# manycore-research/PlankAssembly

Hardware: AMD Instinct MI355X
Metric: train samples/sec (fwd+bwd+all-reduce+Adam), d_model=512 seq=1024 [value: bf16 MFMA, f32 accumulate / master weights; train.f32 / train.x3: the same step in exact f32 / f32 with bf16x3 products = the parity paths] (higher is better)
Workload: dtype bf16; 1 GPU; train_complete.yaml model d_model=512 H=8 dff=1024 6+6 post-norm layers, dropout 0.2, S=1024 (MAX_INPUT_LENGTH 1025), T=128, batch 16/GPU; global_batch=16, seq_len=1024, parallelism=dp1

## Files before the change

### include/plank_hip.h

```cpp
#ifndef PLANK_HIP_H
#define PLANK_HIP_H
#include <stdint.h>

#ifdef __cplusplus
extern "C" {
#endif

#define PA_F32 0
#define PA_BF16 1

#define PA_EINVAL (-1)
#define PA_EALIGN (-2)
#define PA_ESHAPE (-3)

int pa_version(void);

typedef struct {
    const void* A; const void* B; void* C;
    const float* bias;
    const void* R;
    const void* aux;
    void* ws;
    int32_t M, N, K;
    int32_t lda, ldb, ldc, ldr, ldaux;
// ... 152 lines not shown
                    int32_t dtype, const pa_reduce_desc* rd, int32_t n_rd, void* stream);


typedef struct {
    const void* q; const void* k; const void* v; void* o;
    float* lse;
    const uint8_t* kpm;
    int32_t B, H, Lq, Lk, dh;
    int32_t ldq, ldk, ldv, ldo;
    int32_t causal;
    float scale;
    float drop_p; uint32_t drop_seed;
    int32_t dtype;
    const void* dout; void* dq; void* dk; void* dv; float* delta;
    int32_t lddo, lddq, lddk, lddv;
    const int32_t* cu_q; const int32_t* cu_k;
    const int32_t* order;
    void* ws; int64_t ws_bytes;
} pa_attn_args;
int pa_attn_fwd(const pa_attn_args* a, void* stream);
int pa_attn_bwd(const pa_attn_args* a, void* stream);
int64_t pa_attn_ws_bytes(int32_t rows_total, int32_t B, int32_t H, int32_t L_max);
int64_t pa_attn_ws_ticket_bytes(int64_t ws_bytes);
int pa_attn_split_config(int32_t on);
int64_t pa_attn_split_taken(int32_t reset);

int pa_gelu_fwd(void* out, const void* pre, int64_t rows, int32_t cols, int32_t ld, int32_t dtype, float drop_p, uint32_t drop_seed,
                void* stream);
int pa_gelu_bwd(void* dpre, const void* dh, const void* pre, int64_t rows, int32_t cols, int32_t ld, int32_t dtype, float drop_p,
                uint32_t drop_seed, void* stream);
int pa_switch_fwd(float* s, const void* h, int32_t dtype, const float* w, const float* b, int64_t rows,
                  int32_t d, void* stream);
int pa_switch_bwd(void* dh, int32_t accumulate, float* dw, float* db, const float* ds, const void* h,
                  int32_t dtype, const float* w, float* partial, int64_t rows, int32_t d, void* stream);
int pa_mixture_nll_fwd(float* stats, float* row_lse, const float* vocab, int32_t ldv, const float* ptr,
                       const float* sw, const int64_t* label, int32_t B, int32_t T, int32_t V, int32_t pad,
                       void* stream);
int pa_mixture_nll_bwd(void* dvocab, void* dptr, int32_t out_dtype, float* dsw, const float* stats,
                       const float* row_lse, const float* vocab, int32_t ldv, const float* ptr, const float* sw,
                       const int64_t* label, int32_t B, int32_t T, int32_t V, int32_t pad, float gscale,
                       void* stream);
int pa_mixture_nll_fwd_fin(float* stats8, float* row_lse, const float* vocab, int32_t ldv, const float* ptr,
                           const float* sw, const int64_t* label, int32_t B, int32_t T, int32_t V, int32_t pad,
                           void* stream);
int pa_mixture_nll_bwd_up(void* dvocab, void* dptr, int32_t out_dtype, float* dsw, const float* stats,
                       const float* row_lse, const float* vocab, int32_t ldv, const float* ptr, const float* sw,
// ... 99 lines not shown
```

### plankassembly_amd/_lib.py

```python
from __future__ import annotations

import ctypes as C
import os

import torch

HERE = os.path.dirname(os.path.abspath(__file__))
LIB_PATH = os.environ.get("PLANK_HIP_LIB") or os.path.join(HERE, "libplank_hip.so")

PA_F32, PA_BF16 = 0, 1
_ERR = {-1: "PA_EINVAL (bad argument)", -2: "PA_EALIGN (misaligned pointer / leading dimension)",
        -3: "PA_ESHAPE (unsupported shape)", -4: "PA_ESTATE (bad model/workspace state)"}


class PlankHipError(RuntimeError):
    pass


class GemmArgs(C.Structure):
    _fields_ = [("A", C.c_void_p), ("B", C.c_void_p), ("C", C.c_void_p), ("bias", C.c_void_p),
                ("R", C.c_void_p), ("aux", C.c_void_p), ("ws", C.c_void_p),
                ("M", C.c_int32), ("N", C.c_int32), ("K", C.c_int32),
                ("lda", C.c_int32), ("ldb", C.c_int32), ("ldc", C.c_int32), ("ldr", C.c_int32),
                ("ldaux", C.c_int32),
# ... 104 lines not shown
            "pa_gemm_recorded_kinds": (I, [P, I]),
            "pa_gemm_recorded_groups": (I, [P, I]),
            "pa_splitk_reduce_many": (I, [P, I, P]),
            "pa_colsum_many": (I, [P, I, I, P]),
            "pa_colsum_ws_floats": (I64, [I, I]),
            "pa_colsum": (I, [P, I, I, I, I, P, I, P, P]),
            "pa_embed_input_fwd": (I, [P, I, P, P, P, I, I64, I, P]),
            "pa_embed_input_bwd": (I, [P, I, P, P, P, P, I, I64, I, P]),
            "pa_embed_segment_bwd": (I, [P, I, P, P, P, P, I, I64, I, P]),
            "pa_pack_rows": (I, [P, I, I, P, P, P]),
            "pa_group_rows": (I, [P, I, P]),
            "pa_embed_output_fwd": (I, [P, I, P, P, P, P, I, I, I, I, I, P]),
            "pa_embed_output_bwd": (I, [P, I, P, P, P, P, I, I, I, I, I, P]),
            "pa_layernorm_ws_floats": (I64, [I64, I]),
            "pa_layernorm_fwd": (I, [P, P, P, P, P, P, I64, I, F, I, P]),
            "pa_layernorm_bwd": (I, [P, P, P, P, P, P, P, P, P, P, P, I64, I, I, F, U, P]),
            "pa_layernorm_bwd_partial": (I, [P, P, P, P, P, P, P, I, P, I64, I, I, F, U, P]),
            "pa_layernorm_bwd_nparts": (I, [I64]),
            "pa_layernorm_finish_many": (I, [P, I, I, P]),
            "pa_attn_fwd": (I, [P, P]),
            "pa_attn_bwd": (I, [P, P]),
            "pa_attn_ws_bytes": (I64, [I, I, I, I]),
            "pa_attn_ws_ticket_bytes": (I64, [I64]),
            "pa_attn_split_config": (I, [I]),
            "pa_attn_split_taken": (I64, [I]),
            "pa_gelu_fwd": (I, [P, P, I64, I, I, I, F, C.c_uint32, P]),
            "pa_gelu_bwd": (I, [P, P, P, I64, I, I, I, F, C.c_uint32, P]),
            "pa_switch_fwd": (I, [P, P, I, P, P, I64, I, P]),
            "pa_switch_bwd": (I, [P, I, P, P, P, P, I, P, P, I64, I, P]),
            "pa_mixture_nll_fwd": (I, [P, P, P, I, P, P, P, I, I, I, I, P]),
            "pa_mixture_nll_bwd": (I, [P, P, I, P, P, P, P, I, P, P, P, I, I, I, I, F, P]),
            "pa_mixture_nll_fwd_fin": (I, [P, P, P, I, P, P, P, I, I, I, I, P]),
            "pa_mixture_nll_bwd_up": (I, [P, P, I, P, P, P, P, I, P, P, P, I, I, I, I, F, P, P]),
            "pa_model_set_upstream": (I, [P, P]),
            "pa_adam_step": (I, [P, P, P, P, P, I64, F, F, F, F, I, F, P]),
            "pa_cast": (I, [P, I, P, I, I64, P]),
            "pa_fake_collective": (I, [P, I64, I, I, F, P]),
            "pa_model_create": (I, [P, P]),
            "pa_model_destroy": (None, [P]),
            "pa_model_num_params": (I, [P]),
            "pa_model_bind": (I, [P, P, P, P]),
            "pa_model_bind_transposed": (I, [P, P]),
            "pa_model_bind_cross_kv_t": (I, [P, P]),
            "pa_transpose_many": (I, [P, I, I, I, P]),
            "pa_model_train_ws_bytes": (I64, [P, I, I, I]),
            "pa_model_train_fwd": (I, [P, P, P, I64, U, I, P, P]),
# ... 67 lines not shown
```

### plankassembly_amd/csrc/attention.hip

```cpp
#include <stdio.h>
#include <atomic>
#include <algorithm>
#include "pa_device.h"
#include "../../include/plank_hip.h"

namespace {

constexpr int NTH = 256;
constexpr int BOWN = 128;
constexpr int BSTR = 64;
constexpr float LOG2E = 1.4426950408889634f;
constexpr float LN2 = 0.6931471805599453f;
constexpr float RESCALE_THR = 8.0f;

__device__ __forceinline__ float fast_exp2(float x) { return __builtin_amdgcn_exp2f(x); }

struct AttnP;
struct AttnP {
    const void* q; const void* k; const void* v; void* o; float* lse; const uint8_t* kpm;
    int B, H, Lq, Lk;
    int ldq, ldk, ldv, ldo;
    int causal; float scale;
    uint32_t drop_thr; float drop_scale; uint32_t drop_seed;
    const void* dout; void* dq; void* dk; void* dv; float* delta;
    int lddo, lddq, lddk, lddv;
    const int32_t* cu_q; const int32_t* cu_k;
    const int32_t* order;
    int balanced;
    int ks_min;
    int parts_q, parts_kv;
    int* sp_tick; char* sp_part; int sp_slots, sp_pmax, sp_kmax;
};
constexpr int SP_BYTES = 64 * 1024;

__device__ __forceinline__ AttnP batch_view(const AttnP& pin, int b, int& qoff, int& koff, int off = 0, int len = -1) {
    AttnP p = pin;
    qoff = b * pin.Lq; koff = b * pin.Lk;
    if (len >= 0 && pin.cu_q == pin.cu_k) { qoff = koff = off; p.Lq = p.Lk = len; return p; }
    if (pin.cu_q) { qoff = pin.cu_q[b]; p.Lq = pin.cu_q[b + 1] - qoff; }
    if (pin.cu_k) { koff = pin.cu_k[b]; p.Lk = pin.cu_k[b + 1] - koff; }
    return p;
}

template <typename T, int DH> struct AT {
    static constexpr int EB = ET<T>::EB, KC = ET<T>::KC;
    static constexpr int NS = DH / KC;
    static constexpr int NDT = (DH + 31) / 32;
    static constexpr int NCHR = DH / EB;
    static constexpr int RBN = DH * sizeof(T);
    static constexpr int RBT = BSTR * sizeof(T);
    static constexpr int NCHT = RBT / 16;
    static constexpr int NAT_BYTES = BSTR * RBN;
    static constexpr int TR_BYTES = DH * RBT;
    static constexpr int NSB = 16 * NCHR;
    static constexpr int NITEM = (2 * NSB + NTH - 1) / NTH;
};
// ... 653 lines not shown
    for (int d = 1; d < 64; d <<= 1) { const int v = __shfl_up(sinc, d); if (lane >= d) sinc += v; }
    if (sinc > pin.sp_slots) np = 1;
    const int t = tq * np;
    int inc = t;
#pragma unroll
    for (int d = 1; d < 64; d <<= 1) { const int v = __shfl_up(inc, d); if (lane >= d) inc += v; }
    const int n = __shfl(inc, 63);
    const int row = j >> 5, pos = j & 31, left = n - (row << 5);
    if (left <= 0) return false;
    const int rowlen = left < 32 ? left : 32;
    if (pos >= rowlen) return false;
    const int k = (row << 5) + ((row & 1) ? rowlen - 1 - pos : pos);
    const int rank = __popcll(__ballot(inc <= k));
    const int local = k - (__shfl(inc, rank) - __shfl(t, rank));
    const int npr = __shfl(np, rank);
    u.nparts = __builtin_amdgcn_readfirstlane(npr);
    u.tile = __builtin_amdgcn_readfirstlane(local / npr);
    u.part = __builtin_amdgcn_readfirstlane(local % npr);
    u.b = __builtin_amdgcn_readfirstlane(__shfl(o, rank));
    u.off = __builtin_amdgcn_readfirstlane(__shfl(c0, rank));
    u.len = __builtin_amdgcn_readfirstlane(__shfl(cl, rank));
    u.slot = __builtin_amdgcn_readfirstlane(((__shfl(sinc, rank) - __shfl(spl, rank)) + u.tile) * 8 + x);
    u.h = x;
    return true;
}
#include "split_merge.h"


template <int DH> struct BT {
    static constexpr int RBN = DH * 2;
    static constexpr int NCHR = RBN / 16;
    static constexpr int NAT = BSTR * RBN;
    static constexpr int NCHUNK = BSTR * NCHR;
    static constexpr int NLD = (NCHUNK + NTH - 1) / NTH;
    static constexpr int NS = DH / 16;
    static constexpr int NDT = (DH + 31) / 32;
};

template <int DH>
__device__ __forceinline__ void glds_nat(char* lds, const bf16* base, int ld, int row0, int nrows, int tid, int wave) {
    using B = BT<DH>;
    constexpr int RPB = (B::RBN >= 256) ? 1 : 256 / B::RBN;
#pragma unroll
    for (int i = 0; i < B::NLD; ++i) {
        const int p = tid + i * NTH;
        if (B::NCHUNK % NTH == 0 || p < B::NCHUNK) {
// ... 909 lines not shown
        m_run = m_new;
    }
    const float inv = l_tot > 0.f ? (DROP ? p.drop_scale : 1.0f) / l_tot : 0.f;
    bf16* Op = reinterpret_cast<bf16*>(p.o) + (size_t)qoff * p.ldo + h * DH;
    store_rows4(Op, p.ldo, qrow, p.Lq, oacc, inv, lane);
    if (g == 0 && qrow < p.Lq && p.lse)
        p.lse[((size_t)b * p.H + h) * pin.Lq + qrow] = l_tot > 0.f ? (m_run + log2f(l_tot)) * LN2 : 0.f;
#ifdef PA_ATTN_TRACE
    asm volatile("s_waitcnt vmcnt(0)" ::: "memory");
    PA_TR(4);
    if (tid == 0 && blockIdx.x < 8192) { pa_attn_trace[blockIdx.x * 8 + 5] = nsteps; pa_attn_trace[blockIdx.x * 8 + 6] = __builtin_amdgcn_s_getreg((4 << 0) | (0 << 6) | (31 << 11)); }
#endif
}

template <bool DROP, int KS>
__device__ __forceinline__ void attn4_dq_body(const AttnP& pin, int bid, char* smem) {
    constexpr int DH = 64, NAT = BT<DH>::NAT, BUF = BL<DH>::BUF, AUX = BL<DH>::AUX;
    const int lane = threadIdx.x & 63, g = lane >> 4;
    const int wave_all = __builtin_amdgcn_readfirstlane(threadIdx.x >> 6);
    const int kh = KS == 2 ? (wave_all >> 3) : 0;
    const int wave = wave_all & 7, tid = threadIdx.x & (NT4 - 1);
    int tile_, h, b, off_ = 0, len_ = -1;
    int part = 0, nparts = 1, slot = 0;
    if (KS == 1 && pin.balanced == 2) {
        SplitUnit su;
        if (!decode_unit_split(pin, pin.cu_q, su, bid)) return;
        tile_ = su.tile; h = su.h; b = su.b; off_ = su.off; len_ = su.len; part = su.part; nparts = su.nparts; slot = su.slot;
    }
    else if (pin.balanced) { if (!decode_block_balanced(pin, pin.cu_q, tile_, h, b, off_, len_, bid)) return; }
    else { decode_block((pin.Lq + BOWN - 1) / BOWN, pin.H, pin.B, tile_, h, b, bid); b = dispatch_batch(pin.order, b); }
    int qoff, koff;
    const AttnP p = batch_view(pin, b, qoff, koff, off_, len_);
    const int q0 = tile_ * BOWN;
    if (q0 >= p.Lq) return;
    const bf16* Qp = reinterpret_cast<const bf16*>(p.q) + (size_t)qoff * p.ldq + h * DH;
    const bf16* Kp = reinterpret_cast<const bf16*>(p.k) + (size_t)koff * p.ldk + h * DH;
    const bf16* Vp = reinterpret_cast<const bf16*>(p.v) + (size_t)koff * p.ldv + h * DH;
    const bf16* dOp = reinterpret_cast<const bf16*>(p.dout) + (size_t)qoff * p.lddo + h * DH;
    const uint8_t* mp = p.kpm ? p.kpm + (size_t)b * pin.Lk : nullptr;
    const int qw0 = q0 + wave * 16, qrow = qw0 + (lane & 15);
    const bool wave_on = qw0 < p.Lq;

    u32x4 qreg[2], doreg[2];
    load_row4(qreg, Qp, p.ldq, qrow, p.Lq, lane);
    load_row4(doreg, dOp, p.lddo, qrow, p.Lq, lane);
    scale_row4(qreg, p.scale * LOG2E);
    const size_t srow = ((size_t)b * p.H + h) * pin.Lq + qrow;
    const float lse2 = (qrow < p.Lq) ? p.lse[srow] * LOG2E : INFINITY;
    const float keep_p = DROP ? 1.0f / p.drop_scale : 1.0f;
// ... 94 lines not shown
                if (DROP) dp = drop_keep2(arow, cq[kb & 1][e], p.drop_thr) ? dp : ndlt;
                sacc[kb][e] = pe * dp;
            }
        }
        mma_tr4<buf * BUF>(dqacc, lb, sacc);
        tile_barrier();
    };
    for (int step = 0; step < nsteps; step += 2) {
        body(step, IC<0>{});
        if (step + 1 < nsteps) body(step + 1, IC<1>{});
    }
    if (KS == 2 && split) {
        f32x4* xo = reinterpret_cast<f32x4*>(smem) + wave * 4 * 64;
        if (kh == 1) {
#pragma unroll
            for (int db = 0; db < 4; ++db) xo[db * 64 + lane] = dqacc[db];
        }
        __syncthreads();
        if (kh == 1) return;
#pragma unroll
        for (int db = 0; db < 4; ++db) dqacc[db] += xo[db * 64 + lane];
    }
    if (KS == 1 && nparts > 1) {
        char* const pbase = pin.sp_part + (size_t)slot * pin.sp_pmax * SP_BYTES;
        const SplitOut so(pbase + (size_t)part * SP_BYTES, SP_BYTES);
#pragma unroll
        for (int db = 0; db < 4; ++db) so.put(db, NT4, dqacc[db]);
        if (!split_arrive(pin.sp_tick + slot, nparts, reinterpret_cast<int*>(smem + 2 * BUF))) return;
        for (int pp = 0; pp < nparts; ++pp) {
            if (pp == part) continue;
#pragma unroll
            for (int db = 0; db < 4; ++db) dqacc[db] += split_get(pbase + (size_t)pp * SP_BYTES, db, NT4, SP_BYTES);
        }
    }
    bf16* dQp = reinterpret_cast<bf16*>(p.dq) + (size_t)qoff * p.lddq + h * DH;
    store_rows4(dQp, p.lddq, qrow, p.Lq, dqacc, p.scale * (DROP ? p.drop_scale : 1.0f), lane);
}

template <bool DROP, int KS>
__global__ __launch_bounds__(NT4 * KS, 4) void attn4_bwd_dq_kernel(AttnP pin) {
    extern __shared__ __attribute__((aligned(256))) char smem[];
    attn4_dq_body<DROP, KS>(pin, blockIdx.x, smem);
}

template <bool DROP, bool CAUSAL, bool SELF_DELTA>
__device__ __forceinline__ void attn4_dkv_body(const AttnP& pin, int bid, char* smem) {
    constexpr int DH = 64, NAT = BT<DH>::NAT, BUF = BL<DH>::BUF, AUX = BL<DH>::AUX;
    const int tid = threadIdx.x, lane = tid & 63, g = lane >> 4;
    const int wave = __builtin_amdgcn_readfirstlane(tid >> 6);
    int tile_, h, b, off_ = 0, len_ = -1;
    int part = 0, nparts = 1, slot = 0;
    if (!SELF_DELTA && pin.balanced == 2) {
        SplitUnit su;
        if (!decode_unit_split(pin, pin.cu_k, su, bid)) return;
        tile_ = su.tile; h = su.h; b = su.b; off_ = su.off; len_ = su.len; part = su.part; nparts = su.nparts; slot = su.slot;
// ... 118 lines not shown
                    const bool keep = drop_keep2(aq[e], ckey, p.drop_thr);
                    pd = keep ? pe : 0.f;
                    x = keep ? x : __uint_as_float(nd4[qb][e]);
                }
                sacc[qb][e] = pd;
                dpacc[qb][e] = pe * x;
            }
        }
        mma_tr4<buf * BUF + NAT>(dvacc, lb, sacc);
        mma_tr4<buf * BUF>(dkacc, lb, dpacc);
        if (more) issue_aux(step + 1, buf ^ 1);
        tile_barrier();
    };
    for (int step = step0; step < nsteps; step += 2) {
        body(step, IC<0>{});
        if (step + 1 < nsteps) body(step + 1, IC<1>{});
    }
    if (nparts > 1) {
        char* const pbase = pin.sp_part + (size_t)slot * pin.sp_pmax * SP_BYTES;
        const SplitOut so(pbase + (size_t)part * SP_BYTES, SP_BYTES);
#pragma unroll
        for (int db = 0; db < 4; ++db) { so.put(db, NT4, dkacc[db]); so.put(4 + db, NT4, dvacc[db]); }
        if (!split_arrive(pin.sp_tick + slot, nparts, reinterpret_cast<int*>(smem + 2 * BUF))) return;
        for (int pp = 0; pp < nparts; ++pp) {
            if (pp == part) continue;
#pragma unroll
            for (int db = 0; db < 4; ++db) {
                dkacc[db] += split_get(pbase + (size_t)pp * SP_BYTES, db, NT4, SP_BYTES);
                dvacc[db] += split_get(pbase + (size_t)pp * SP_BYTES, 4 + db, NT4, SP_BYTES);
            }
        }
    }
    bf16* dKp = reinterpret_cast<bf16*>(p.dk) + (size_t)koff * p.lddk + h * DH;
    bf16* dVp = reinterpret_cast<bf16*>(p.dv) + (size_t)koff * p.lddv + h * DH;
    const float ds = DROP ? p.drop_scale : 1.0f;
    store_rows4(dKp, p.lddk, krow, p.Lk, dkacc, kmasked ? 0.f : p.scale * ds, lane, kmasked);
    store_rows4(dVp, p.lddv, krow, p.Lk, dvacc, kmasked ? 0.f : ds, lane, kmasked);
}

template <bool DROP, bool CAUSAL>
__global__ __launch_bounds__(NT4, 4) void attn4_bwd_dkv_kernel(AttnP pin) {
    extern __shared__ __attribute__((aligned(256))) char smem[];
    attn4_dkv_body<DROP, CAUSAL, false>(pin, blockIdx.x, smem);
}
template <bool DROP, bool CAUSAL>
__global__ __launch_bounds__(NT4, 4) void attn4_bwd_merged_kernel(AttnP pin, int gq) {
    extern __shared__ __attribute__((aligned(256))) char smem[];
    if ((int)blockIdx.x < gq) attn4_dq_body<DROP, 1>(pin, blockIdx.x, smem);
    else attn4_dkv_body<DROP, CAUSAL, true>(pin, (int)blockIdx.x - gq, smem);
}

#include "attention5.h"
#include "attention_x3.h"

static int split_kmax() { static const int v = getenv("PA_ATTN_SPLIT_KMAX") ? atoi(getenv("PA_ATTN_SPLIT_KMAX")) : 8; return v < 1 ? 1 : v; }
static int split_pmax() { static const int v = getenv("PA_ATTN_SPLIT_PMAX") ? atoi(getenv("PA_ATTN_SPLIT_PMAX")) : 2; return v < 1 ? 1 : v > 8 ? 8 : v; }
AttnP make_params(const pa_attn_args* a) {
    AttnP p;
    p.q = a->q; p.k = a->k; p.v = a->v; p.o = a->o; p.lse = a->lse; p.kpm = a->kpm;
    p.B = a->B; p.H = a->H; p.Lq = a->Lq; p.Lk = a->Lk;
    p.ldq = a->ldq; p.ldk = a->ldk; p.ldv = a->ldv; p.ldo = a->ldo;
    p.causal = a->causal; p.scale = a->scale;
    p.drop_thr = (uint32_t)((double)a->drop_p * 4294967296.0);
    p.drop_scale = (float)(1.0 / (1.0 - (double)p.drop_thr / 4294967296.0));
    p.drop_seed = a->drop_seed;
    p.dout = a->dout; p.dq = a->dq; p.dk = a->dk; p.dv = a->dv; p.delta = a->delta;
    p.lddo = a->lddo; p.lddq = a->lddq; p.lddk = a->lddk; p.lddv = a->lddv;
    p.cu_q = a->cu_q; p.cu_k = a->cu_k; p.order = a->order;
    static const bool bal_env = !(getenv("PA_ATTN_BALANCED") && atoi(getenv("PA_ATTN_BALANCED")) == 0);
    p.ks_min = 4; p.parts_q = 1; p.parts_kv = 1;
    p.balanced = (bal_env && a->order && a->cu_q && a->cu_k && a->H == 8 && a->B <= 64) ? 1 : 0;
    p.sp_tick = nullptr; p.sp_part = nullptr; p.sp_slots = 0; p.sp_pmax = split_pmax(); p.sp_kmax = split_kmax();
    static const bool sp_env = getenv("PA_ATTN_SPLIT") && atoi(getenv("PA_ATTN_SPLIT")) != 0;
    if (sp_env && p.balanced && a->ws && a->cu_q == a->cu_k && !a->kpm && !a->causal && a->dtype == PA_BF16 && a->dh == 64 &&
        (reinterpret_cast<uintptr_t>(a->ws) & 255) == 0 && p.sp_pmax > 1) {
        const int64_t per = (int64_t)p.sp_pmax * SP_BYTES + 64;
        const int64_t total = a->ws_bytes / per;
        p.sp_slots = (int)(total / 8 < (1 << 20) ? total / 8 : (1 << 20));
        p.sp_tick = static_cast<int*>(a->ws);
        p.sp_part = static_cast<char*>(a->ws) + ((int64_t)p.sp_slots * 8 * 4 + 255) / 256 * 256;
        if ((int64_t)p.sp_slots * 8 * per > a->ws_bytes || p.sp_slots < 1) { p.sp_slots = 0; p.sp_tick = nullptr; }
    }
    return p;
}
static unsigned split_grid(const AttnP& p, int owned_max, int streamed_max) {
    const int ks = (streamed_max + BSTR - 1) / BSTR;
    const int np = ks > p.sp_kmax ? std::min(p.sp_pmax, (ks + p.sp_kmax - 1) / p.sp_kmax) : 1;
    return (unsigned)(8 * p.B * ((owned_max + BOWN - 1) / BOWN) * np);
}

template <typename K> int set_lds(K kern, int bytes) {
    if (bytes > 64 * 1024) {
        hipError_t e = hipFuncSetAttribute(reinterpret_cast<const void*>(kern), hipFuncAttributeMaxDynamicSharedMemorySize, bytes);
        if (e != hipSuccess) return (int)e;
    }
    return 0;
}

static bool use_v4(const AttnP& p, int rows_owned) {
    static const int mode = getenv("PA_ATTN_V4") ? atoi(getenv("PA_ATTN_V4")) : 1;
    if (mode == 0) return false;
    if (mode >= 2) return true;
    const long long waves32 = (long long)p.B * p.H * ((rows_owned + 31) / 32);
    return p.cu_q != nullptr || p.cu_k != nullptr || waves32 < 4 * 1024;
}
// ... 36 lines not shown
                if (p.drop_thr) PA_LAUNCH((attn4_fwd_kernel<true, 2>), grid, dim3(2 * NT4), shm2, st, p);
                else PA_LAUNCH((attn4_fwd_kernel<false, 2>), grid, dim3(2 * NT4), shm2, st, p);
                return 0;
            }
            if (p.drop_thr) PA_LAUNCH((attn4_fwd_kernel<true, 1>), grid, dim3(NT4), shm, st, p);
            else PA_LAUNCH((attn4_fwd_kernel<false, 1>), grid, dim3(NT4), shm, st, p);
            return 0;
        }
    }
    if (p.drop_thr) PA_LAUNCH((attn_fwd_bf16_kernel<DH, true>), grid, dim3(NTH), shm, st, p);
    else PA_LAUNCH((attn_fwd_bf16_kernel<DH, false>), grid, dim3(NTH), shm, st, p);
    return 0;
}
template <int DH> int run_bwd_bf16(AttnP p, hipStream_t st) {
    const int shm = BL<DH>::SHM;
    const dim3 gq0(((p.Lq + BOWN - 1) / BOWN) * p.H * p.B), gk0(((p.Lk + BOWN - 1) / BOWN) * p.H * p.B);
    if constexpr (DH == 64) {
        if (use_v4(p, p.Lq > p.Lk ? p.Lq : p.Lk)) {
            dim3 gq = gq0, gk = gk0;
            static const bool merge_env = !(getenv("PA_ATTN_BWD_MERGE") && atoi(getenv("PA_ATTN_BWD_MERGE")) == 0);
            static const int merge_max = getenv("PA_ATTN_BWD_MERGE_MAX") ? atoi(getenv("PA_ATTN_BWD_MERGE_MAX")) : 128;
            if (merge_env && p.Lq <= merge_max && p.Lq <= 2048 && (gq.x & 7) == 0) {
                const int shm3 = shm + (p.Lq + 15) / 16 * 64 + 64;
                const dim3 gm(gq.x + gk.x);
                if (p.drop_thr) {
                    if (p.causal) PA_LAUNCH((attn4_bwd_merged_kernel<true, true>), gm, dim3(NT4), shm3, st, p, (int)gq.x);
                    else PA_LAUNCH((attn4_bwd_merged_kernel<true, false>), gm, dim3(NT4), shm3, st, p, (int)gq.x);
                } else {
                    if (p.causal) PA_LAUNCH((attn4_bwd_merged_kernel<false, true>), gm, dim3(NT4), shm3, st, p, (int)gq.x);
                    else PA_LAUNCH((attn4_bwd_merged_kernel<false, false>), gm, dim3(NT4), shm3, st, p, (int)gq.x);
                }
                return 0;
            }
            bool ks = use_ksplit(p, gq.x);
            constexpr int shm2 = 4 * BL<DH>::BUF + 64;
            if (p.balanced && p.sp_tick && !ks) { p.balanced = 2; gq = dim3(split_grid(p, p.Lq, p.Lk)); gk = dim3(split_grid(p, p.Lk, p.Lq)); }
            if (ks) {
                static const int rc_d = set_lds(attn4_bwd_dq_kernel<true, 2>, shm2), rc_n = set_lds(attn4_bwd_dq_kernel<false, 2>, shm2);
                if (rc_d || rc_n) return rc_d ? rc_d : rc_n;
            }
            if (p.drop_thr) {
                if (ks) PA_LAUNCH((attn4_bwd_dq_kernel<true, 2>), gq, dim3(2 * NT4), shm2, st, p);
                else PA_LAUNCH((attn4_bwd_dq_kernel<true, 1>), gq, dim3(NT4), shm, st, p);
                if (p.causal) PA_LAUNCH((attn4_bwd_dkv_kernel<true, true>), gk, dim3(NT4), shm, st, p);
                else PA_LAUNCH((attn4_bwd_dkv_kernel<true, false>), gk, dim3(NT4), shm, st, p);
            } else {
                if (ks) PA_LAUNCH((attn4_bwd_dq_kernel<false, 2>), gq, dim3(2 * NT4), shm2, st, p);
                else PA_LAUNCH((attn4_bwd_dq_kernel<false, 1>), gq, dim3(NT4), shm, st, p);
                if (p.causal) PA_LAUNCH((attn4_bwd_dkv_kernel<false, true>), gk, dim3(NT4), shm, st, p);
                else PA_LAUNCH((attn4_bwd_dkv_kernel<false, false>), gk, dim3(NT4), shm, st, p);
            }
            return 0;
        }
    }
    const dim3 gq = gq0, gk = gk0;
    static const int occ_env = getenv("PA_ATTN_OCC") ? atoi(getenv("PA_ATTN_OCC")) : 0;
// ... 108 lines not shown
    if (bwd) {
        if (!a->dout || !a->dq || !a->dk || !a->dv || !a->delta) return PA_EINVAL;
        if (!al(a->dout, a->lddo) || !al(a->dq, a->lddq) || !al(a->dk, a->lddk) || !al(a->dv, a->lddv)) return PA_EALIGN;
    }
    return 0;
}

}

extern "C" int pa_attn_split_config(int32_t on) { return pa_split_attn_set(on); }
extern "C" int64_t pa_attn_split_taken(int32_t reset) {
    const long long v = g_attn_x3_taken.load();
    if (reset) g_attn_x3_taken.store(0);
    return v;
}

extern "C" int64_t pa_attn_ws_bytes(int32_t rows_total, int32_t B, int32_t H, int32_t L_max) {
    static const bool sp_env = getenv("PA_ATTN_SPLIT") && atoi(getenv("PA_ATTN_SPLIT")) != 0;
    if (!sp_env || split_pmax() < 2 || H != 8 || rows_total <= 0 || B <= 0 || B > 64) return 0;
    if ((L_max + BSTR - 1) / BSTR <= split_kmax()) return 0;
    const int64_t slots = (int64_t)(rows_total / BOWN + B);
    return slots * 8 * ((int64_t)split_pmax() * SP_BYTES + 64) + 256;
}
extern "C" int64_t pa_attn_ws_ticket_bytes(int64_t ws_bytes) {
    const int64_t per = (int64_t)split_pmax() * SP_BYTES + 64;
    return (ws_bytes / per / 8 * 8 * 4 + 255) / 256 * 256;
}

extern "C" int pa_attn_fwd(const pa_attn_args* a, void* stream) {
    int rc = check_args(a, false);
    if (rc) return rc;
    hipStream_t st = reinterpret_cast<hipStream_t>(stream);
    return a->dtype == PA_BF16 ? dispatch<bf16>(a, false, st) : dispatch<float>(a, false, st);
}

extern "C" int pa_attn_bwd(const pa_attn_args* a, void* stream) {
    int rc = check_args(a, true);
    if (rc) return rc;
    hipStream_t st = reinterpret_cast<hipStream_t>(stream);
    return a->dtype == PA_BF16 ? dispatch<bf16>(a, true, st) : dispatch<float>(a, true, st);
}

#ifdef PA_ATTN_TRACE
extern "C" int pa_attn_trace_read(unsigned long long* out, int32_t n) {
    return (int)hipMemcpyFromSymbol(out, HIP_SYMBOL(pa_attn_trace), sizeof(unsigned long long) * (size_t)n);
}
// ... 2 lines not shown
```

### plankassembly_amd/csrc/model.h

```cpp
#pragma once
#include <hip/hip_runtime.h>
#include <stdint.h>
#include <vector>
#include "../../include/plank_hip.h"

struct Arena {
    char* base; size_t off;
    void* take(size_t bytes) {
        size_t o = (off + 255) & ~(size_t)255;
        off = o + bytes;
        return base ? base + o : nullptr;
    }
};

static inline uint32_t site_seed(uint32_t base, uint32_t site) {
    uint32_t x = base + 0x9e3779b9u * (site + 1);
    x ^= x >> 16; x *= 0x7feb352du; x ^= x >> 15; x *= 0x846ca68bu; x ^= x >> 16;
    return x;
}

enum { P_IN_VALUE = 0, P_IN_POS, P_IN_COORD, P_IN_VIEW, P_IN_TYPE, P_Q_COORD, P_Q_POS, P_FIXED_HEAD };
enum { E_IN_W = 0, E_IN_B, E_OUT_W, E_OUT_B, E_L1_W, E_L1_B, E_L2_W, E_L2_B, E_N1_W, E_N1_B, E_N2_W, E_N2_B, E_COUNT };
enum { D_SA_IN_W = 0, D_SA_IN_B, D_SA_OUT_W, D_SA_OUT_B, D_CA_IN_W, D_CA_IN_B, D_CA_OUT_W, D_CA_OUT_B,
       D_L1_W, D_L1_B, D_L2_W, D_L2_B, D_N1_W, D_N1_B, D_N2_W, D_N2_B, D_N3_W, D_N3_B, D_COUNT };
// ... 6 lines not shown
    void *qkv, *o_sa, *z1, *y1, *q_ca, *kv_ca, *o_ca, *z2, *y2, *hff, *z3;
    int ld_kv = 0;
    float *lse_sa, *lse_ca, *m1, *r1, *m2, *r2, *m3, *r3;
};

struct DecodeLayout;
struct pa_model {
    pa_model_cfg cfg;
    int n_params;
    std::vector<void*> pf, pl, gr;
    std::vector<void*> plT;
    bool bound = false;
    bool have_fwd = false;
    pa_batch batch;
    int B = 0, S = 0, T = 0;
    int NE = 0;
    uint32_t seed = 0; float p_drop = 0.f;
    size_t esz = 4;
    std::vector<void*> X, Y;
    std::vector<EncAct> ea; std::vector<DecAct> da;
    void *memory = nullptr, *hid = nullptr; float *mem_m = nullptr, *mem_r = nullptr, *hid_m = nullptr, *hid_r = nullptr;
    float *vlog = nullptr, *plog = nullptr, *sw = nullptr, *row_lse = nullptr; void* pfeat = nullptr; int ldv = 0;
    float* stats = nullptr;
    void* attn_ws = nullptr; int64_t attn_ws_bytes = 0; void* attn_ws_zeroed = nullptr; int64_t attn_ws_zeroed_bytes = 0;
    const float* upstream = nullptr;
    void *gA, *gB, *gC, *gD, *gE, *gF, *gQ3, *gKV, *dmem, *dvlog, *dplog; float *dsw, *delta, *partial, *splitws;
    void* gPre = nullptr;
    size_t splitws_floats = 0;
    void* gBs[3] = {nullptr, nullptr, nullptr}; void* gCs[3] = {nullptr, nullptr, nullptr};
    float* lnp[3] = {nullptr, nullptr, nullptr}; pa_ln_finish_desc lnq[PA_MAX_LN_FINISH]; int nlnq = 0;
    pa_gemm_args dwq[PA_MAX_GROUP]; int ndwq = 0;
    pa_colsum_desc cs[PA_MAX_COLSUM]; int ncs = 0; bool defer_ok = false;
    pa_reduce_desc defer[PA_MAX_REDUCE]; int ndefer = 0; size_t slab_used = 0;
    bool dmem_written = false;
    void* kv_all = nullptr;
    void* gKV_all = nullptr; const void* kvT_all = nullptr;
    struct SegSet { void* gBs[3]; void* gCs[3]; void *gE, *gF, *gQ3, *gKV; float* lnp[3]; float* splitws; };
    SegSet seg_set[2];
    void select_set(int par) {
        const SegSet& s = seg_set[par];
        for (int i = 0; i < 3; ++i) { gBs[i] = s.gBs[i]; gCs[i] = s.gCs[i]; lnp[i] = s.lnp[i]; }
        gE = s.gE; gF = s.gF; gQ3 = s.gQ3; gKV = s.gKV; splitws = s.splitws;
    }
    bool side_on = false;
    void* side = nullptr;
    void* ev_ready[2] = {nullptr, nullptr};
    void* ev_done[2] = {nullptr, nullptr};
// ... 12 lines not shown
```

### plankassembly_amd/csrc/runtime.hip

```cpp
#include <stdlib.h>
#include <hip/hip_runtime.h>
#include <math.h>
#include <new>
#include <string.h>
#include <vector>
#include "../../include/plank_hip.h"

#include "model.h"

namespace {

#define RC(x) do { int rc_ = (x); if (rc_) return rc_; } while (0)

struct Ctx {
    pa_model* m; void* st;
    int dt() const { return m->cfg.dtype; }
    bool gelu() const { return m->cfg.activation == 2; }
    int ffn1(const void* A, const void* W, const float* bias, void* hidden, int rows, float drop_p, uint32_t seed) const {
        const int d = m->cfg.d_model, ff = m->cfg.d_ff;
        if (!gelu()) return linear(A, d, W, bias, hidden, ff, rows, ff, d, 1, drop_p, seed);
        RC(linear(A, d, W, bias, hidden, ff, rows, ff, d, 0));
        return pa_gelu_fwd(hidden, hidden, rows, ff, ff, dt(), drop_p, seed, st);
    }

// ... 102 lines not shown
            void* const out = ddrop ? ddrop : dz;
            const bool al = ((reinterpret_cast<uintptr_t>(dz) | reinterpret_cast<uintptr_t>(dy) | reinterpret_cast<uintptr_t>(z) |
                              reinterpret_cast<uintptr_t>(ddrop) | reinterpret_cast<uintptr_t>(g) | reinterpret_cast<uintptr_t>(part)) & 15) == 0;
            void* img = (al && pa_layernorm_bwd_can_img(m->cfg.d_model, dt())) ?
                        pa_gemm_split_reserve(out, (int32_t)rows, m->cfg.d_model, m->cfg.d_model, &pat) : nullptr;
            RC(pa_layernorm_bwd_partial_img(dz, ddrop, dy, z, g, mean, rstd, dzsum ? 1 : 0, part, rows, m->cfg.d_model, dt(), drop_p, seed,
                                            img, pat, st));
            pa_ln_finish_desc& fd = m->lnq[m->nlnq++];
            fd.partial = part; fd.nparts = pa_layernorm_bwd_nparts(rows); fd.pad_ = 0; fd.dgamma = dg; fd.dbeta = db; fd.dzsum = dzsum;
            return 0;
        }
        return pa_layernorm_bwd(dz, ddrop, dy, z, g, mean, rstd, dg, db, dzsum, m->partial, rows, m->cfg.d_model, dt(),
                                drop_p, seed, st);
    }
    int attn(bool bwd, const void* q, int ldq, const void* k, const void* v, int ldkv, void* o, float* lse,
             const uint8_t* kpm, int Lq, int Lk, int causal, float drop_p, uint32_t seed,
             const void* dout = nullptr, void* dq = nullptr, int lddq = 0, void* dk = nullptr, void* dv = nullptr,
             int lddkv = 0, const int32_t* cu_q = nullptr, const int32_t* cu_k = nullptr) const {
        pa_attn_args a; memset(&a, 0, sizeof(a));
        a.cu_q = cu_q; a.cu_k = cu_k;
        static const bool use_order = !(getenv("PA_ATTN_ORDER") && atoi(getenv("PA_ATTN_ORDER")) == 0);
        if (use_order && cu_k && cu_k == m->batch.cu_in) a.order = cu_k + m->B + 1;
        if (cu_q && cu_q == cu_k) { a.ws = m->attn_ws; a.ws_bytes = m->attn_ws_bytes; }
        const int d = m->cfg.d_model, H = m->cfg.n_head;
        a.q = q; a.k = k; a.v = v; a.o = o; a.lse = lse; a.kpm = kpm;
        a.B = m->B; a.H = H; a.Lq = Lq; a.Lk = Lk; a.dh = d / H;
        a.ldq = ldq; a.ldk = ldkv; a.ldv = ldkv; a.ldo = d;
        a.causal = causal; a.scale = 1.0f / sqrtf((float)(d / H));
        a.drop_p = drop_p; a.drop_seed = seed; a.dtype = dt();
        if (!bwd) return pa_attn_fwd(&a, st);
        a.dout = dout; a.dq = dq; a.dk = dk; a.dv = dv; a.delta = m->delta;
        a.lddo = d; a.lddq = lddq; a.lddk = lddkv; a.lddv = lddkv;
        return pa_attn_bwd(&a, st);
    }
};

}
size_t pa_train_layout(pa_model* m, char* base, int B, int S, int T) {
    const pa_model_cfg& c = m->cfg;
    const size_t e = c.dtype == PA_BF16 ? 2 : 4;
    const size_t d = c.d_model, ff = c.d_ff, H = c.n_head;
    const size_t BS = (size_t)B * S, BT = (size_t)B * T, R = BS > BT ? BS : BT;
    Arena a{base, 0};
    m->esz = e;
    {
        const int64_t n = c.dtype == PA_BF16 ? pa_attn_ws_bytes(B * S, B, (int32_t)H, S) : 0;
        m->attn_ws = n > 0 ? a.take((size_t)n) : nullptr;
        m->attn_ws_bytes = n > 0 ? n : 0;
    }
    m->X.resize(c.n_enc + 1); m->Y.resize(c.n_dec + 1); m->ea.resize(c.n_enc); m->da.resize(c.n_dec);
    for (int i = 0; i <= c.n_enc; ++i) m->X[i] = a.take(BS * d * e);
    for (int i = 0; i < c.n_enc; ++i) {
        EncAct& t = m->ea[i];
        t.qkv = a.take(BS * 3 * d * e); t.o = a.take(BS * d * e); t.z1 = a.take(BS * d * e); t.y1 = a.take(BS * d * e);
        t.hff = a.take(BS * ff * e); t.z2 = a.take(BS * d * e);
        t.lse = (float*)a.take((size_t)B * H * S * 4);
        t.m1 = (float*)a.take(BS * 4); t.r1 = (float*)a.take(BS * 4); t.m2 = (float*)a.take(BS * 4); t.r2 = (float*)a.take(BS * 4);
    }
    m->memory = a.take(BS * d * e); m->mem_m = (float*)a.take(BS * 4); m->mem_r = (float*)a.take(BS * 4);
    for (int i = 0; i <= c.n_dec; ++i) m->Y[i] = a.take(BT * d * e);
    for (int i = 0; i < c.n_dec; ++i) {
        DecAct& t = m->da[i];
        t.qkv = a.take(BT * 3 * d * e); t.o_sa = a.take(BT * d * e); t.z1 = a.take(BT * d * e); t.y1 = a.take(BT * d * e);
        t.q_ca = a.take(BT * d * e); t.kv_ca = nullptr; t.o_ca = a.take(BT * d * e);
        t.z2 = a.take(BT * d * e); t.y2 = a.take(BT * d * e); t.hff = a.take(BT * ff * e); t.z3 = a.take(BT * d * e);
        t.lse_sa = (float*)a.take((size_t)B * H * T * 4); t.lse_ca = (float*)a.take((size_t)B * H * T * 4);
        t.m1 = (float*)a.take(BT * 4); t.r1 = (float*)a.take(BT * 4); t.m2 = (float*)a.take(BT * 4);
        t.r2 = (float*)a.take(BT * 4); t.m3 = (float*)a.take(BT * 4); t.r3 = (float*)a.take(BT * 4);
// ... 503 lines not shown

extern "C" int64_t pa_model_train_ws_bytes(pa_model* m, int32_t B, int32_t S, int32_t T) {
    if (!m || B <= 0 || S <= 0 || T <= 0) return PA_EINVAL;
    return (int64_t)pa_train_layout(m, nullptr, B, S, T) + 256;
}

extern "C" int pa_model_train_fwd(pa_model* m, const pa_batch* batch, void* ws, int64_t ws_bytes, uint32_t seed,
                                  int32_t training, float* stats, void* stream) {
    if (!m || !m->bound || !batch || !ws || !stats) return PA_EINVAL;
    if (batch->B <= 0 || batch->S <= 0 || batch->T <= 0 || !batch->input_idx[0] || !batch->input_mask) return PA_EINVAL;
    if (batch->output_value && (!batch->output_label || !batch->output_mask)) return PA_EINVAL;
    if ((reinterpret_cast<uintptr_t>(ws) & 255) != 0) return PA_EALIGN;
    const size_t need = pa_train_layout(m, (char*)ws, batch->B, batch->S, batch->T);
    if ((int64_t)need > ws_bytes) return PA_EINVAL;
    m->batch = *batch; m->B = batch->B; m->S = batch->S; m->T = batch->T;
    if (batch->cu_in) {
        if (!batch->rowmap || batch->n_valid <= 0 || batch->n_valid > batch->B * batch->S) return PA_EINVAL;
        m->NE = batch->n_valid;
    } else {
        m->NE = batch->B * batch->S;
    }
    m->seed = seed; m->p_drop = training ? m->cfg.dropout : 0.f;
    m->stats = stats;
    if (m->attn_ws && (m->attn_ws != m->attn_ws_zeroed || m->attn_ws_bytes != m->attn_ws_zeroed_bytes)) {
        if (hipMemsetAsync(m->attn_ws, 0, (size_t)pa_attn_ws_ticket_bytes(m->attn_ws_bytes), (hipStream_t)stream) != hipSuccess) return PA_EINVAL;
        m->attn_ws_zeroed = m->attn_ws; m->attn_ws_zeroed_bytes = m->attn_ws_bytes;
    }
    m->have_fwd = false;
    int rc = pa_train_forward_impl(m, stream);
    if (rc == 0) m->have_fwd = batch->output_value != nullptr;
    return rc;
}

extern "C" int pa_model_set_upstream(pa_model* m, const float* upstream) {
    if (!m) return PA_EINVAL;
    m->upstream = upstream;
    return 0;
}
extern "C" int32_t pa_model_stats_floats(void) { return PA_MODEL_STATS_FLOATS; }
extern "C" int pa_model_train_num_segments(const pa_model* m) {
    return m ? m->cfg.n_dec + m->cfg.n_enc + 4 : PA_EINVAL;
}

extern "C" int pa_model_train_bwd(pa_model* m, int32_t seg_lo, int32_t seg_hi, float gscale, void* stream) {
    if (!m || !m->have_fwd) return PA_EINVAL;
    for (int i = 0; i < m->n_params; ++i) if (!m->gr[i]) return PA_EINVAL;
    const int nseg = m->cfg.n_dec + m->cfg.n_enc + 4;
    if (seg_lo < 0 || seg_hi > nseg || seg_lo > seg_hi) return PA_EINVAL;
    for (int s = seg_lo; s < seg_hi; ++s) RC(backward_segment(m, s, gscale, stream));
    if (seg_hi == nseg && m->side_on) { RC(join_side(m, 0, stream)); RC(join_side(m, 1, stream)); m->select_set(0); }
// ... 23 lines not shown
```

### plankassembly_amd/ops.py

```python
from __future__ import annotations

import ctypes as C
import math

import torch

from . import _lib as L


def _f32(*shape, device):
    return torch.empty(*shape, dtype=torch.float32, device=device)


def gemm(a, b, *, a_kcontig=True, b_kcontig=True, bias=None, residual=None, aux=None, aux_scale=1.0,
         relu=False, alpha=1.0, drop_p=0.0, drop_seed=0, out_dtype=None, splitk=1, out=None, defer=False, out_lp=None):
    batched = a.dim() == 3
    A3 = a if batched else a[None]
    B3 = b if b.dim() == 3 else b[None]
    batch = A3.shape[0]
    M, K = (A3.shape[1], A3.shape[2]) if a_kcontig else (A3.shape[2], A3.shape[1])
    N = B3.shape[1] if b_kcontig else B3.shape[2]
    assert (B3.shape[2] if b_kcontig else B3.shape[1]) == K
    assert A3.stride(2) == 1 and B3.stride(2) == 1
    out_dtype = out_dtype or a.dtype
# ... 318 lines not shown
                                       L.ptr(vocab), vocab.stride(-2), L.ptr(ptr), L.ptr(sw), L.ptr(label), B, T, V,
                                       pad, C.c_float(gscale), L.stream()), "pa_mixture_nll_bwd")
    return dvocab, dptr, dsw


def adam_step(p, g, m, v, step, lr=1e-4, b1=0.9, b2=0.999, eps=1e-8, gscale=1.0, p_bf16=None):
    L.check(L.lib().pa_adam_step(L.ptr(p), L.ptr(g), L.ptr(m), L.ptr(v), L.ptr(p_bf16), C.c_int64(p.numel()),
                                 C.c_float(lr), C.c_float(b1), C.c_float(b2), C.c_float(eps), int(step),
                                 C.c_float(gscale), L.stream()), "pa_adam_step")


def cast(src, dtype):
    dst = torch.empty(src.shape, dtype=dtype, device=src.device)
    L.check(L.lib().pa_cast(L.ptr(dst), L.dt(dst), L.ptr(src), L.dt(src), C.c_int64(src.numel()), L.stream()),
            "pa_cast")
    return dst


def attn_split_ws(rows_total, B, H, device, L_max=1 << 20):
    n = int(L.lib().pa_attn_ws_bytes(int(rows_total), int(B), int(H), int(L_max)))
    return torch.zeros(n, dtype=torch.uint8, device=device) if n > 0 else None


def attn_varlen_fwd(q, k, v, H, cu_q, cu_k, B, Lq_max, Lk_max, causal=False, scale=None, drop_p=0.0, drop_seed=0, order=None, ws=None):
    o = torch.empty(q.shape[0], q.shape[1], dtype=q.dtype, device=q.device)
    lse = _f32(B, H, Lq_max, device=q.device)
    a = _attn_args(q, k, v, o, lse, None, causal, scale, drop_p, drop_seed, H, cu_q, cu_k, B, Lq_max, Lk_max, order)
    if ws is not None:
        a.ws, a.ws_bytes = ws.data_ptr(), ws.numel()
    L.check(L.lib().pa_attn_fwd(C.byref(a), L.stream()), "pa_attn_fwd")
    return o, lse


def attn_varlen_bwd(dout, q, k, v, o, lse, H, cu_q, cu_k, B, Lq_max, Lk_max, causal=False, scale=None, drop_p=0.0, drop_seed=0, order=None, ws=None):
    a = _attn_args(q, k, v, o, lse, None, causal, scale, drop_p, drop_seed, H, cu_q, cu_k, B, Lq_max, Lk_max, order)
    if ws is not None:
        a.ws, a.ws_bytes = ws.data_ptr(), ws.numel()
    dq = torch.empty(q.shape, dtype=q.dtype, device=q.device)
    dk = torch.empty(k.shape, dtype=k.dtype, device=k.device)
    dv = torch.empty(v.shape, dtype=v.dtype, device=v.device)
    delta = _f32(lse.shape, device=q.device)
    a.dout, a.dq, a.dk, a.dv, a.delta = dout.data_ptr(), dq.data_ptr(), dk.data_ptr(), dv.data_ptr(), delta.data_ptr()
    a.lddo, a.lddq, a.lddk, a.lddv = dout.stride(-2), dq.stride(-2), dk.stride(-2), dv.stride(-2)
    L.check(L.lib().pa_attn_bwd(C.byref(a), L.stream()), "pa_attn_bwd")
    return dq, dk, dv

# ... 36 lines not shown
```

Measured before the change: 3261 samples/s.

## Split cross-attention backward dQ over key-length partitions with ticketed merge

Adds a cross-attention split path for the merged backward kernel: when queries are short (T≤128) and keys are long, each (batch, head) dQ tile is split across up to four key-range partitions, and a ticket counter merges the partial sums. This gives more workgroups to fill the GPU, where otherwise only B*H blocks run over the long key sequence. The merge now sums the partitions in a fixed order so the result is deterministic. A dedicated workspace and a per-step memset of the tickets are added; the old skip of the self-attention ticket memset is removed, so that memset now runs every step.

```diff
diff --git a/include/plank_hip.h b/include/plank_hip.h
--- a/include/plank_hip.h
+++ b/include/plank_hip.h
@@ -198,6 +198,8 @@
 int pa_attn_bwd(const pa_attn_args* a, void* stream);
 int64_t pa_attn_ws_bytes(int32_t rows_total, int32_t B, int32_t H, int32_t L_max);
 int64_t pa_attn_ws_ticket_bytes(int64_t ws_bytes);
+int64_t pa_attn_cross_ws_bytes(int32_t B, int32_t H, int32_t Lq, int32_t Lk);
+int64_t pa_attn_cross_ws_ticket_bytes(int32_t B, int32_t H);
 int pa_attn_split_config(int32_t on);
 int64_t pa_attn_split_taken(int32_t reset);
 
diff --git a/plankassembly_amd/_lib.py b/plankassembly_amd/_lib.py
--- a/plankassembly_amd/_lib.py
+++ b/plankassembly_amd/_lib.py
@@ -150,6 +150,8 @@
             "pa_attn_bwd": (I, [P, P]),
             "pa_attn_ws_bytes": (I64, [I, I, I, I]),
             "pa_attn_ws_ticket_bytes": (I64, [I64]),
+            "pa_attn_cross_ws_bytes": (I64, [I, I, I, I]),
+            "pa_attn_cross_ws_ticket_bytes": (I64, [I, I]),
             "pa_attn_split_config": (I, [I]),
             "pa_attn_split_taken": (I64, [I]),
             "pa_gelu_fwd": (I, [P, P, I64, I, I, I, F, C.c_uint32, P]),
diff --git a/plankassembly_amd/csrc/attention.hip b/plankassembly_amd/csrc/attention.hip
--- a/plankassembly_amd/csrc/attention.hip
+++ b/plankassembly_amd/csrc/attention.hip
@@ -30,8 +30,10 @@
     int ks_min;
     int parts_q, parts_kv;
     int* sp_tick; char* sp_part; int sp_slots, sp_pmax, sp_kmax;
+    int xsplit, sp_stride;
 };
 constexpr int SP_BYTES = 64 * 1024;
+constexpr int SPQ_BYTES = 32 * 1024;
 
 __device__ __forceinline__ AttnP batch_view(const AttnP& pin, int b, int& qoff, int& koff, int off = 0, int len = -1) {
     AttnP p = pin;
@@ -731,6 +733,27 @@
     u.len = __builtin_amdgcn_readfirstlane(__shfl(cl, rank));
     u.slot = __builtin_amdgcn_readfirstlane(((__shfl(sinc, rank) - __shfl(spl, rank)) + u.tile) * 8 + x);
     u.h = x;
+    return true;
+}
+__device__ __forceinline__ bool decode_unit_cross(const AttnP& pin, SplitUnit& u, int L) {
+    const int x = L & 7, j = L >> 3;
+    const int lane = threadIdx.x & 63;
+    int o = 0, np = 0;
+    if (lane < pin.B) {
+        o = pin.order ? pin.order[lane] : lane;
+        const int ks = (pin.cu_k[o + 1] - pin.cu_k[o] + BSTR - 1) / BSTR;
+        np = ks > pin.sp_kmax ? min(pin.sp_pmax, (ks + pin.sp_kmax - 1) / pin.sp_kmax) : 1;
+    }
+    int inc = np;
+#pragma unroll
+    for (int d = 1; d < 64; d <<= 1) { const int v = __shfl_up(inc, d); if (lane >= d) inc += v; }
+    if (j >= __shfl(inc, 63)) return false;
+    const int rank = __popcll(__ballot(inc <= j));
+    u.nparts = __builtin_amdgcn_readfirstlane(__shfl(np, rank));
+    u.part = __builtin_amdgcn_readfirstlane(j - (__shfl(inc, rank) - u.nparts));
+    u.b = __builtin_amdgcn_readfirstlane(__shfl(o, rank));
+    u.slot = __builtin_amdgcn_readfirstlane(rank * 8 + x);
+    u.tile = 0; u.h = x; u.off = 0; u.len = -1;
     return true;
 }
 #include "split_merge.h"
@@ -1686,9 +1709,9 @@
     const int wave = wave_all & 7, tid = threadIdx.x & (NT4 - 1);
     int tile_, h, b, off_ = 0, len_ = -1;
     int part = 0, nparts = 1, slot = 0;
-    if (KS == 1 && pin.balanced == 2) {
+    if (KS == 1 && (pin.xsplit || pin.balanced == 2)) {
         SplitUnit su;
-        if (!decode_unit_split(pin, pin.cu_q, su, bid)) return;
+        if (!(pin.xsplit ? decode_unit_cross(pin, su, bid) : decode_unit_split(pin, pin.cu_q, su, bid))) return;
         tile_ = su.tile; h = su.h; b = su.b; off_ = su.off; len_ = su.len; part = su.part; nparts = su.nparts; slot = su.slot;
     }
     else if (pin.balanced) { if (!decode_block_balanced(pin, pin.cu_q, tile_, h, b, off_, len_, bid)) return; }
@@ -1829,15 +1852,27 @@
         for (int db = 0; db < 4; ++db) dqacc[db] += xo[db * 64 + lane];
     }
     if (KS == 1 && nparts > 1) {
-        char* const pbase = pin.sp_part + (size_t)slot * pin.sp_pmax * SP_BYTES;
-        const SplitOut so(pbase + (size_t)part * SP_BYTES, SP_BYTES);
+        const int pstride = pin.sp_stride;
+        char* const pbase = pin.sp_part + (size_t)slot * pin.sp_pmax * pstride;
+        const SplitOut so(pbase + (size_t)part * pstride, SPQ_BYTES);
 #pragma unroll
         for (int db = 0; db < 4; ++db) so.put(db, NT4, dqacc[db]);
         if (!split_arrive(pin.sp_tick + slot, nparts, reinterpret_cast<int*>(smem + 2 * BUF))) return;
-        for (int pp = 0; pp < nparts; ++pp) {
-            if (pp == part) continue;
-#pragma unroll
-            for (int db = 0; db < 4; ++db) dqacc[db] += split_get(pbase + (size_t)pp * SP_BYTES, db, NT4, SP_BYTES);
+        f32x4 own[4];
+#pragma unroll
+        for (int db = 0; db < 4; ++db) own[db] = dqacc[db];
+        if (part != 0) {
+#pragma unroll
+            for (int db = 0; db < 4; ++db) dqacc[db] = split_get(pbase, db, NT4, SPQ_BYTES);
+        }
+        for (int pp = 1; pp < nparts; ++pp) {
+            if (pp == part) {
+#pragma unroll
+                for (int db = 0; db < 4; ++db) dqacc[db] += own[db];
+            } else {
+#pragma unroll
+                for (int db = 0; db < 4; ++db) dqacc[db] += split_get(pbase + (size_t)pp * pstride, db, NT4, SPQ_BYTES);
+            }
         }
     }
     bf16* dQp = reinterpret_cast<bf16*>(p.dq) + (size_t)qoff * p.lddq + h * DH;
@@ -2002,12 +2037,23 @@
 #pragma unroll
         for (int db = 0; db < 4; ++db) { so.put(db, NT4, dkacc[db]); so.put(4 + db, NT4, dvacc[db]); }
         if (!split_arrive(pin.sp_tick + slot, nparts, reinterpret_cast<int*>(smem + 2 * BUF))) return;
-        for (int pp = 0; pp < nparts; ++pp) {
-            if (pp == part) continue;
-#pragma unroll
-            for (int db = 0; db < 4; ++db) {
-                dkacc[db] += split_get(pbase + (size_t)pp * SP_BYTES, db, NT4, SP_BYTES);
-                dvacc[db] += split_get(pbase + (size_t)pp * SP_BYTES, 4 + db, NT4, SP_BYTES);
+        f32x4 ownk[4], ownv[4];
+#pragma unroll
+        for (int db = 0; db < 4; ++db) { ownk[db] = dkacc[db]; ownv[db] = dvacc[db]; }
+        if (part != 0) {
+#pragma unroll
+            for (int db = 0; db < 4; ++db) { dkacc[db] = split_get(pbase, db, NT4, SP_BYTES); dvacc[db] = split_get(pbase, 4 + db, NT4, SP_BYTES); }
+        }
+        for (int pp = 1; pp < nparts; ++pp) {
+            if (pp == part) {
+#pragma unroll
+                for (int db = 0; db < 4; ++db) { dkacc[db] += ownk[db]; dvacc[db] += ownv[db]; }
+            } else {
+#pragma unroll
+                for (int db = 0; db < 4; ++db) {
+                    dkacc[db] += split_get(pbase + (size_t)pp * SP_BYTES, db, NT4, SP_BYTES);
+                    dvacc[db] += split_get(pbase + (size_t)pp * SP_BYTES, 4 + db, NT4, SP_BYTES);
+                }
             }
         }
     }
@@ -2035,6 +2081,15 @@
 
 static int split_kmax() { static const int v = getenv("PA_ATTN_SPLIT_KMAX") ? atoi(getenv("PA_ATTN_SPLIT_KMAX")) : 8; return v < 1 ? 1 : v; }
 static int split_pmax() { static const int v = getenv("PA_ATTN_SPLIT_PMAX") ? atoi(getenv("PA_ATTN_SPLIT_PMAX")) : 2; return v < 1 ? 1 : v > 8 ? 8 : v; }
+static bool xsplit_on() { static const bool v = !(getenv("PA_ATTN_XSPLIT") && atoi(getenv("PA_ATTN_XSPLIT")) == 0); return v; }
+static int xsplit_kmax() { static const int v = getenv("PA_ATTN_XSPLIT_KMAX") ? atoi(getenv("PA_ATTN_XSPLIT_KMAX")) : 8; return v < 1 ? 1 : v; }
+static int xsplit_pmax() { static const int v = getenv("PA_ATTN_XSPLIT_PMAX") ? atoi(getenv("PA_ATTN_XSPLIT_PMAX")) : 4; return v < 1 ? 1 : v > 8 ? 8 : v; }
+static int xsplit_parts(int Lk) {
+    const int ks = (Lk + BSTR - 1) / BSTR;
+    return ks > xsplit_kmax() ? std::min(xsplit_pmax(), (ks + xsplit_kmax() - 1) / xsplit_kmax()) : 1;
+}
+static int64_t xsplit_ticket_bytes(int B, int H) { return ((int64_t)B * H * 4 + 255) / 256 * 256; }
+extern "C" int pa_get_reserved_cus(void);
 AttnP make_params(const pa_attn_args* a) {
     AttnP p;
     p.q = a->q; p.k = a->k; p.v = a->v; p.o = a->o; p.lse = a->lse; p.kpm = a->kpm;
@@ -2061,6 +2116,16 @@
         p.sp_part = static_cast<char*>(a->ws) + ((int64_t)p.sp_slots * 8 * 4 + 255) / 256 * 256;
         if ((int64_t)p.sp_slots * 8 * per > a->ws_bytes || p.sp_slots < 1) { p.sp_slots = 0; p.sp_tick = nullptr; }
     }
+    p.xsplit = 0; p.sp_stride = SP_BYTES;
+    if (xsplit_on() && !a->cu_q && a->cu_k && a->ws && !a->kpm && !a->causal && a->dtype == PA_BF16 && a->dh == 64 && a->H == 8 &&
+        a->B <= 64 && a->Lq <= BOWN && (reinterpret_cast<uintptr_t>(a->ws) & 255) == 0 && xsplit_parts(a->Lk) > 1 &&
+        a->B * a->H <= 256 - pa_get_reserved_cus() &&
+        a->ws_bytes >= xsplit_ticket_bytes(a->B, a->H) + (int64_t)a->B * a->H * xsplit_pmax() * SPQ_BYTES) {
+        p.xsplit = 1; p.sp_stride = SPQ_BYTES; p.sp_kmax = xsplit_kmax(); p.sp_slots = a->B * a->H;
+        p.sp_pmax = xsplit_parts(a->Lk);
+        p.sp_tick = static_cast<int*>(a->ws);
+        p.sp_part = static_cast<char*>(a->ws) + xsplit_ticket_bytes(a->B, a->H);
+    }
     return p;
 }
 static unsigned split_grid(const AttnP& p, int owned_max, int streamed_max) {
@@ -2143,6 +2208,7 @@
             static const int merge_max = getenv("PA_ATTN_BWD_MERGE_MAX") ? atoi(getenv("PA_ATTN_BWD_MERGE_MAX")) : 128;
             if (merge_env && p.Lq <= merge_max && p.Lq <= 2048 && (gq.x & 7) == 0) {
                 const int shm3 = shm + (p.Lq + 15) / 16 * 64 + 64;
+                if (p.xsplit) gq = dim3(gq.x * xsplit_parts(p.Lk));
                 const dim3 gm(gq.x + gk.x);
                 if (p.drop_thr) {
                     if (p.causal) PA_LAUNCH((attn4_bwd_merged_kernel<true, true>), gm, dim3(NT4), shm3, st, p, (int)gq.x);
@@ -2153,6 +2219,7 @@
                 }
                 return 0;
             }
+            p.xsplit = 0;
             bool ks = use_ksplit(p, gq.x);
             constexpr int shm2 = 4 * BL<DH>::BUF + 64;
             if (p.balanced && p.sp_tick && !ks) { p.balanced = 2; gq = dim3(split_grid(p, p.Lq, p.Lk)); gk = dim3(split_grid(p, p.Lk, p.Lq)); }
@@ -2307,6 +2374,12 @@
     const int64_t slots = (int64_t)(rows_total / BOWN + B);
     return slots * 8 * ((int64_t)split_pmax() * SP_BYTES + 64) + 256;
 }
+extern "C" int64_t pa_attn_cross_ws_bytes(int32_t B, int32_t H, int32_t Lq, int32_t Lk) {
+    if (!xsplit_on() || H != 8 || B <= 0 || B > 64 || Lq <= 0 || Lq > BOWN || xsplit_parts(Lk) < 2) return 0;
+    if (B * H > 256 - pa_get_reserved_cus()) return 0;
+    return xsplit_ticket_bytes(B, H) + (int64_t)B * H * xsplit_pmax() * SPQ_BYTES;
+}
+extern "C" int64_t pa_attn_cross_ws_ticket_bytes(int32_t B, int32_t H) { return xsplit_ticket_bytes(B, H); }
 extern "C" int64_t pa_attn_ws_ticket_bytes(int64_t ws_bytes) {
     const int64_t per = (int64_t)split_pmax() * SP_BYTES + 64;
     return (ws_bytes / per / 8 * 8 * 4 + 255) / 256 * 256;
diff --git a/plankassembly_amd/csrc/model.h b/plankassembly_amd/csrc/model.h
--- a/plankassembly_amd/csrc/model.h
+++ b/plankassembly_amd/csrc/model.h
@@ -52,7 +52,8 @@
     void *memory = nullptr, *hid = nullptr; float *mem_m = nullptr, *mem_r = nullptr, *hid_m = nullptr, *hid_r = nullptr;
     float *vlog = nullptr, *plog = nullptr, *sw = nullptr, *row_lse = nullptr; void* pfeat = nullptr; int ldv = 0;
     float* stats = nullptr;
-    void* attn_ws = nullptr; int64_t attn_ws_bytes = 0; void* attn_ws_zeroed = nullptr; int64_t attn_ws_zeroed_bytes = 0;
+    void* xattn_ws = nullptr; int64_t xattn_ws_bytes = 0;
+    void* attn_ws = nullptr; int64_t attn_ws_bytes = 0;
     const float* upstream = nullptr;
     void *gA, *gB, *gC, *gD, *gE, *gF, *gQ3, *gKV, *dmem, *dvlog, *dplog; float *dsw, *delta, *partial, *splitws;
     void* gPre = nullptr;
diff --git a/plankassembly_amd/csrc/runtime.hip b/plankassembly_amd/csrc/runtime.hip
--- a/plankassembly_amd/csrc/runtime.hip
+++ b/plankassembly_amd/csrc/runtime.hip
@@ -148,6 +148,7 @@
         static const bool use_order = !(getenv("PA_ATTN_ORDER") && atoi(getenv("PA_ATTN_ORDER")) == 0);
         if (use_order && cu_k && cu_k == m->batch.cu_in) a.order = cu_k + m->B + 1;
         if (cu_q && cu_q == cu_k) { a.ws = m->attn_ws; a.ws_bytes = m->attn_ws_bytes; }
+        else if (bwd && !cu_q && cu_k) { a.ws = m->xattn_ws; a.ws_bytes = m->xattn_ws_bytes; }
         const int d = m->cfg.d_model, H = m->cfg.n_head;
         a.q = q; a.k = k; a.v = v; a.o = o; a.lse = lse; a.kpm = kpm;
         a.B = m->B; a.H = H; a.Lq = Lq; a.Lk = Lk; a.dh = d / H;
@@ -170,6 +171,9 @@
     Arena a{base, 0};
     m->esz = e;
     {
+        const int64_t nx = c.dtype == PA_BF16 && d / H == 64 ? pa_attn_cross_ws_bytes(B, (int32_t)H, T, S) : 0;
+        m->xattn_ws = nx > 0 ? a.take((size_t)nx) : nullptr;
+        m->xattn_ws_bytes = nx > 0 ? nx : 0;
         const int64_t n = c.dtype == PA_BF16 ? pa_attn_ws_bytes(B * S, B, (int32_t)H, S) : 0;
         m->attn_ws = n > 0 ? a.take((size_t)n) : nullptr;
         m->attn_ws_bytes = n > 0 ? n : 0;
@@ -719,10 +723,8 @@
     }
     m->seed = seed; m->p_drop = training ? m->cfg.dropout : 0.f;
     m->stats = stats;
-    if (m->attn_ws && (m->attn_ws != m->attn_ws_zeroed || m->attn_ws_bytes != m->attn_ws_zeroed_bytes)) {
-        if (hipMemsetAsync(m->attn_ws, 0, (size_t)pa_attn_ws_ticket_bytes(m->attn_ws_bytes), (hipStream_t)stream) != hipSuccess) return PA_EINVAL;
-        m->attn_ws_zeroed = m->attn_ws; m->attn_ws_zeroed_bytes = m->attn_ws_bytes;
-    }
+    if (m->xattn_ws && hipMemsetAsync(m->xattn_ws, 0, (size_t)pa_attn_cross_ws_ticket_bytes(m->B, m->cfg.n_head), (hipStream_t)stream) != hipSuccess) return PA_EINVAL;
+    if (m->attn_ws && hipMemsetAsync(m->attn_ws, 0, (size_t)pa_attn_ws_ticket_bytes(m->attn_ws_bytes), (hipStream_t)stream) != hipSuccess) return PA_EINVAL;
     m->have_fwd = false;
     int rc = pa_train_forward_impl(m, stream);
     if (rc == 0) m->have_fwd = batch->output_value != nullptr;
diff --git a/plankassembly_amd/ops.py b/plankassembly_amd/ops.py
--- a/plankassembly_amd/ops.py
+++ b/plankassembly_amd/ops.py
@@ -364,6 +364,11 @@
     return torch.zeros(n, dtype=torch.uint8, device=device) if n > 0 else None
 
 
+def attn_cross_ws(B, H, Lq, Lk, device):
+    n = int(L.lib().pa_attn_cross_ws_bytes(int(B), int(H), int(Lq), int(Lk)))
+    return torch.zeros(n, dtype=torch.uint8, device=device) if n > 0 else None
+
+
 def attn_varlen_fwd(q, k, v, H, cu_q, cu_k, B, Lq_max, Lk_max, causal=False, scale=None, drop_p=0.0, drop_seed=0, order=None, ws=None):
     o = torch.empty(q.shape[0], q.shape[1], dtype=q.dtype, device=q.device)
     lse = _f32(B, H, Lq_max, device=q.device)
```

Measured after the change: 3260 samples/s. Within noise of the previous version (-0.0%).
